# Cons-Cat/Pixel-Art-Raytracer

Measured on AMD Instinct MI355X. Metric: Mrays/sec at 4096x4096, 1024 prims, higher is better.
Workload: dtype int32+f32; 1 GPU; 4096x4096x4096 view, bin 40, 1024 primitives (splitmix64 seed 12345), light (2560,2048,1024); RGBA8 frame + palette-index plane; frames_in_flight=4, streams_overlap_pairwise=True

## Files before the change

pixel-art-raytracer_amd/csrc/par_book.cpp:

```cpp
#include "par_book.h"
#include "par_internal.h"

using S = par_book_state;

static par_footprint footprint_of(const par_book& b, const par_aabb& a) {
    const int W = b.W, H = b.H, L = b.L, B = b.B;
    par_footprint f;
    const int minx = a.px, miny = a.py, minz = a.pz;
    const int maxx = minx + a.ex, maxy = miny + a.ey, maxz = minz + a.ez;
    if ((maxx < 0) || (minx >= W) || (maxy < 0 - maxz) || (miny >= H - minz + B) || (maxz < -a.ez - B) ||
        (minz > L + B)) {
        return f;
    }
    const int x0 = std::max(0, minx / B), y0 = std::max(0, (H - maxy - maxz) / B), z0 = std::max(0, minz / B);
    const int x1 = std::min(b.gx, (maxx + B - 1) / B), y1 = std::min(b.gy, (H - miny - minz + B - 1) / B);
    const int z1 = std::min(b.gz, (maxz + B - 1) / B);
    if (x1 <= x0 || y1 <= y0 || z1 <= z0) return f;
    f.x0 = (int16_t)x0; f.x1 = (int16_t)x1; f.y0 = (int16_t)y0; f.y1 = (int16_t)y1;
    f.nz = z1 - z0;
    f.items = (int32_t)((int)a.ex * ((int)a.ey + (int)a.ez) / 64 + f.cols());
    f.px = a.px; f.ex = a.ex;
    f.row0 = H - ((int)a.py + a.ey + a.pz + a.ez);
    f.rh = (int)a.ey + (int)a.ez;
    return f;
// ... 45 lines not shown
        exact += fp[i].bound();
    }
    rebuild_hist();
}

const par_book_plan& par_book::plan(par_change kind, const par_aabb* a, int first, int n) {
    refresh(kind == par_change::UPDATE ? S::CURRENT : kind == par_change::STAGE ? S::HIST_BEHIND : S::EXTENTS_ONLY);
    par_book_plan& p = plan_;
    const bool whole = kind == par_change::SET;
    p.kind = kind; p.aabbs = a; p.first = first; p.n = n;
    par_bound ex = whole ? par_bound{0, 0, 0} : exact, et = whole ? par_bound{0, 0, 0} : extent;
    const par_aabb* old = whole ? nullptr : aabbs.data() + first;
    if (kind != par_change::ASYNC) {
        p.fp.resize((size_t)n);
        par_footprint* out = p.fp.data();
        for (int i = 0; i < n; i++) {
            const par_footprint f = footprint_of(*this, a[i]);
            out[i] = f;
            ex += f.bound();
            if (old) ex -= fp[(size_t)(first + i)].bound();
        }
    }
    for (int i = 0; i < n; i++) {
        if (old && old[i].ex == a[i].ex && old[i].ey == a[i].ey && old[i].ez == a[i].ez) continue;
        et += bound_of(*this, a[i]);
        if (old) et -= bound_of(*this, old[i]);
    }
    p.exact = ex; p.extent = et;
    if (kind == par_change::ASYNC) ex = et;
    p.need = par_bound{std::max(ex.pairs, et.pairs), std::max(ex.cols, et.cols), std::max(ex.items, et.items)};
    return p;
}

void par_book::commit() {
    par_book_plan& p = plan_;
    if (p.kind != par_change::ASYNC) exact = p.exact;
    extent = p.extent;
    if (p.kind == par_change::SET) {
        aabbs.assign(p.aabbs, p.aabbs + p.n);
        fp.swap(p.fp);
        return rebuild_hist();
    }
    std::copy(p.aabbs, p.aabbs + p.n, aabbs.begin() + p.first);
    if (p.kind == par_change::UPDATE) {
        for (int i = 0; i < p.n; i++) {
            col_hist(fp[(size_t)(p.first + i)], -1);
            col_hist(p.fp[(size_t)i], +1);
        }
    }
    if (p.kind != par_change::ASYNC) std::copy(p.fp.begin(), p.fp.begin() + p.n, fp.begin() + p.first);
    state = std::max(state, p.kind == par_change::UPDATE  ? S::CURRENT
                            : p.kind == par_change::STAGE ? S::HIST_BEHIND : S::EXTENTS_ONLY);
}

const par_bound& par_book::capture() {
    refresh(S::CURRENT);
    const int64_t pairs = exact.pairs * 2 + 4096;
    const int64_t cols_max = (int64_t)((PAR_SPRITE_W + B - 1) / B + 1) * ((PAR_SPRITE_H + B - 1) / B + 1);
    const int64_t items = (int64_t)aabbs.size() * ((int64_t)PAR_SPRITE_W * PAR_SPRITE_H / 64 + cols_max);
    return graph = par_bound{pairs, pairs, std::min(items, max_items())};
}

int64_t par_book::items_per_shard(int64_t items, int64_t cols) const {
    cols = std::min<int64_t>(cols, (int64_t)gx * gy);
    return std::min(items, (cols / PAR_ITEM_SHARDS + 1) * tile_chunks());
}
```

pixel-art-raytracer_amd/csrc/par_book.h:

```cpp
#ifndef PAR_BOOK_H
#define PAR_BOOK_H

#include <stdint.h>
#include <algorithm>
#include <vector>

#include "par_raytracer.h"

struct par_bound {
    int64_t pairs, cols, items;
    par_bound& operator+=(const par_bound& b) { pairs += b.pairs; cols += b.cols; items += b.items; return *this; }
    par_bound& operator-=(const par_bound& b) { pairs -= b.pairs; cols -= b.cols; items -= b.items; return *this; }
};

struct par_footprint {
    int16_t x0 = 0, x1 = 0, y0 = 0, y1 = 0;
    int32_t nz = 0;
    int32_t items = 0;
    int16_t px = 0, ex = 0;
    int32_t row0 = 0, rh = 0;
    int32_t cols() const { return (x1 - x0) * (y1 - y0); }
    par_bound bound() const { return par_bound{(int64_t)cols() * nz, cols(), items}; }
};

enum class par_book_state : uint8_t { CURRENT, HIST_BEHIND, EXTENTS_ONLY };

enum class par_change : uint8_t { SET, UPDATE, STAGE, ASYNC };

struct par_book_plan {
    par_change kind = par_change::SET;
    const par_aabb* aabbs = nullptr; int first = 0, n = 0;
    par_bound exact{}, extent{};
    par_bound need{};
    std::vector<par_footprint> fp;
};

struct par_book {
    int W = 0, H = 0, L = 0, B = 0, gx = 0, gy = 0, gz = 0;
    par_book_state state = par_book_state::CURRENT;
    std::vector<par_aabb> aabbs;
    std::vector<par_footprint> fp;
    par_bound exact{};
    par_bound extent{};
    par_bound graph{};
    std::vector<int32_t> colpairs;
    int64_t cols_over = 0;
    std::vector<int32_t> colchunks;
    int64_t cols_tileable = 0;
    par_book_plan plan_;

    void init(const par_params& p, int x, int y, int z) {
        W = p.width; H = p.height; L = p.length; B = p.bin_size; gx = x; gy = y; gz = z;
    }
    const par_book_plan& plan(par_change kind, const par_aabb* a, int first, int n);
    void commit();
    void refresh(par_book_state lag);
    const par_bound& capture();
    void col_hist(const par_footprint& f, int sign);
    void rebuild_hist();

    par_bound frame_bounds(bool graph_mode) const {
        return graph_mode ? graph : state == par_book_state::EXTENTS_ONLY ? extent : exact;
    }
    bool may_overflow() const { return cols_over > 0 || state != par_book_state::CURRENT; }
    bool dense() const { return cols_tileable >= std::max<int64_t>(16, (int64_t)gx * gy / 64); }
    int64_t chunks() const { return std::min(exact.items, max_items()); }
    int64_t tile_chunks() const { return ((int64_t)B * B + 63) / 64; }
    int64_t max_items() const { return (int64_t)gx * gy * tile_chunks(); }
    int64_t items_per_shard(int64_t items, int64_t cols) const;
};

#endif
```

pixel-art-raytracer_amd/csrc/par_context.hip:

```cpp
#include <algorithm>
#include <array>
#include <cmath>
#include <new>
#include <cstdio>
#include <cstdlib>
#include <cstring>
#include <string>
#include <unordered_map>
#include <vector>

#include "par_book.h"
#include "par_hostcall.h"
#include "par_internal.h"

struct par_context {
    par_params params{};
    int device = 0;
    int gx = 0, gy = 0, gz = 0, volume = 0;
    hipStream_t stream = nullptr;

    par_book book;
    int n_entities = 0, n_sprites = 0, max_sprite_id = 0;
    bool have_entities = false;
    par_light lights[PAR_MAX_LIGHTS]{};
    int n_lights = 0;
    int depth_min = 0, depth_max = 0;
    int light_model = PAR_LIGHTS_UNBOUNDED;
    bool tinted = false;
    par_light_tints tints{};
    int set = 0;
    struct {
        bool valid = false;
        int r0 = 0, r1 = 0, set = 0;
        bool host_gbuf = false;
    } kept;
    struct {
        bool valid = false;
        const void* fb = nullptr;
        const void* palidx = nullptr;
        int r0 = 0, r1 = 0, set = 0;
    } drawn;
    hipStream_t last_stream = nullptr;
    bool has_last_stream = false;

    par_aabb* d_aabbs = nullptr;
    int32_t* d_sprite_ids = nullptr;
    par_sprite* d_sprites = nullptr;
    par_color* d_palette = nullptr;
    par_texel* d_texinfo = nullptr;
    unsigned long long* d_ray_counter = nullptr;
    uint8_t* d_scratch_lit = nullptr;
    size_t scratch_lit_bytes = 0;
    par_grid_dev grid{};
    int aabb_capacity = 0;

    uint8_t* d_out[5] = {nullptr, nullptr, nullptr, nullptr, nullptr};
    size_t d_out_bytes[5] = {0, 0, 0, 0, 0};

    hipGraphExec_t graph_exec[2] = {nullptr, nullptr};
    hipGraph_t graph[2] = {nullptr, nullptr};
    par_aabb* pin_aabbs[2] = {nullptr, nullptr};
    int pin_aabbs_capacity[2] = {0, 0};
    par_lights_block* pin_lights[2] = {nullptr, nullptr};
    hipEvent_t ev_graph[2] = {nullptr, nullptr};
    bool ev_graph_pending[2] = {false, false};
    int stage_lo[2] = {0, 0}, stage_hi[2] = {0, 0};
    int dev_lo = 0, dev_hi = 0;
    par_aabb* pin_update = nullptr;
    int pin_update_capacity = 0;
    hipEvent_t ev_update = nullptr;
    bool ev_update_pending = false;
    hipStream_t update_stream = nullptr;
    bool graph_lights = false;
    par_lights_block* d_lights = nullptr;
// ... 44 lines not shown

void test_alloc_hook(const par_context* c) {
    if (c->hooks & PAR_HOOK_BAD_ALLOC) throw std::bad_alloc();
}

template <class F>
int guarded(par_context* ctx, F&& body) noexcept {
    try {
        return body();
    } catch (const std::bad_alloc&) {
        return fail(ctx, PAR_ERR_OOM, "host allocation failed");
    } catch (...) {
        return fail(ctx, PAR_ERR_HIP, "unexpected C++ exception");
    }
}

void retain_frame(par_context* c, int row_begin, int row_end, int set, bool host_gbuf) {
    c->kept.valid = true;
    c->kept.r0 = row_begin;
    c->kept.r1 = row_end;
    c->kept.set = set;
    c->kept.host_gbuf = host_gbuf;
}
void drop_retained(par_context* c) { c->kept.valid = false; }

void record_drawn(par_context* c, const par_outputs& out, int row_begin, int row_end, int set) {
    c->drawn.valid = true;
    c->drawn.fb = out.fb;
    c->drawn.palidx = out.palidx;
    c->drawn.r0 = row_begin;
    c->drawn.r1 = row_end;
    c->drawn.set = set;
}
void drop_drawn(par_context* c) { c->drawn.valid = false; }

int hip_fail(par_context* c, hipError_t e, const char* what) {
    return fail(c, e == hipErrorOutOfMemory ? PAR_ERR_OOM : PAR_ERR_HIP,
                std::string(what) + ": " + hipGetErrorString(e));
}

#define PAR_HIP(call)                                        \
    do {                                                     \
        hipError_t e_ = (call);                              \
        if (e_ != hipSuccess) return hip_fail(ctx, e_, #call); \
    } while (0)

bool extent_ok(const par_aabb& a) {
    return a.ex >= 0 && a.ey >= 0 && a.ez >= 0 && a.ex <= PAR_SPRITE_W && (int)a.ey + (int)a.ez <= PAR_SPRITE_H;
}

int check_update(par_context* ctx, const par_aabb* aabbs, int first, int n, bool null_ok) {
    if (first < 0 || n < 0 || !ctx->have_entities || first + n > ctx->n_entities || (!aabbs && !(null_ok && n == 0))) {
        return fail(ctx, PAR_ERR_INVALID_ARG, null_ok ? "stage range" : "update range outside the uploaded entities");
    }
    for (int i = 0; i < n; i++) {
        if (!extent_ok(aabbs[i])) return fail(ctx, PAR_ERR_EXTENT, "extent needs 0<=ex<=20, ey,ez>=0, ey+ez<=40");
    }
    return PAR_OK;
}

template <class T>
hipError_t reallocate(T** p, size_t n, bool pinned = false) {
    if (*p) {
        const hipError_t e = pinned ? hipHostFree(*p) : hipFree(*p);
        if (e != hipSuccess) return e;
    }
    *p = nullptr;
// ... 222 lines not shown
    }
    return PAR_OK;
}

int enqueue_lights_frame(par_context* ctx, hipStream_t stream, const par_bin_args& b, const par_render_args& r,
                         const par_bound& bound, bool graph_mode, bool apart, hipEvent_t* ev) {
    const par_light_state lights = make_light_state(ctx, graph_mode);
    const int rc = enqueue_build(ctx, stream, b, bound.pairs, &r, nullptr, apart);
    if (rc != PAR_OK) return rc;
    if (ev) {
        PAR_HIP(hipEventRecord(ev[EV_BUILT], stream));
        PAR_HIP(hipEventRecord(ev[EV_COLUMNS], stream));
    }
    if (r.trace_bg) PAR_HIP(par_launch_bglights(ctx->grid, r, lights, stream));
    PAR_HIP(par_launch_fill(ctx->grid, r, stream));
    if (ev) PAR_HIP(hipEventRecord(ev[EV_FILLED], stream));
    PAR_HIP(par_launch_render_lights(ctx->grid, r, lights, bound.cols, stream));
    if (ev) {
        PAR_HIP(hipEventRecord(ev[EV_ITEMS], stream));
        PAR_HIP(hipEventRecord(ev[EV_RENDERED], stream));
        PAR_HIP(hipEventRecord(ev[EV_END], stream));
        ctx->timed_tiles = false;
        ctx->timed_overflow = false;
        ctx->timed_both = false;
    }
    return PAR_OK;
}

int enqueue_frame(par_context* ctx, hipStream_t stream, int set, int row_begin, int row_end, const par_outputs& out,
                  unsigned flags, bool graph_mode, hipEvent_t* ev) {
    const bool drawn_match = ctx->drawn.valid && ctx->drawn.fb == out.fb && ctx->drawn.palidx == out.palidx &&
                             ctx->drawn.r0 == row_begin && ctx->drawn.r1 == row_end && ctx->drawn.set == (set ^ 1);
    drop_retained(ctx);
    drop_drawn(ctx);
    par_outputs outs = out;
    if ((flags & PAR_RENDER_TRACE_BACKGROUND) && !outs.lit) {
        const size_t need = (size_t)(row_end - row_begin) * ctx->params.width;
        if (ctx->scratch_lit_bytes < need) {
            if (graph_mode) return fail(ctx, PAR_ERR_NOT_READY, "render once with PAR_RENDER_TRACE_BACKGROUND before capturing it");
            PAR_HIP(grow(&ctx->d_scratch_lit, &ctx->scratch_lit_bytes, need));
        }
        outs.lit = ctx->d_scratch_lit;
    }
    if (ctx->ev_update_pending && ctx->update_stream != stream && !graph_mode) {
        PAR_HIP(hipStreamWaitEvent(stream, ctx->ev_update, 0));
    }
    if (ctx->dev_hi > ctx->dev_lo && !graph_mode) {
        PAR_HIP(hipMemcpyAsync(ctx->d_aabbs + ctx->dev_lo, ctx->book.aabbs.data() + ctx->dev_lo,
                               (size_t)(ctx->dev_hi - ctx->dev_lo) * sizeof(par_aabb), hipMemcpyHostToDevice, stream));
        ctx->dev_lo = ctx->dev_hi = 0;
    }
    par_bin_args b = make_bin_args(ctx, set, row_begin, row_end, flags);
    par_render_args r = make_render_args(ctx, set, row_begin, row_end, outs, flags, graph_mode);
    const bool apart = ev && !(flags & PAR_RENDER_TIMED_AS_LAUNCHED);
    const par_bound bound = ctx->book.frame_bounds(graph_mode);
    if ((flags & PAR_RENDER_COUNT_RAYS) && !graph_mode) {
        PAR_HIP(hipMemsetAsync(ctx->d_ray_counter, 0, 3 * sizeof(unsigned long long), stream));
    }
    if (ev) PAR_HIP(hipEventRecord(ev[EV_START], stream));
    if (graph_mode ? ctx->graph_lights : lights_path(ctx)) {
        return enqueue_lights_frame(ctx, stream, b, r, bound, graph_mode, apart, ev);
    }
    const bool may_overflow = graph_mode || ctx->book.may_overflow() || r.dense || apart;
    r.overflow_launched = may_overflow ? 1 : 0;
    par_fill_plan plan;
    const bool ride = !apart && par_plan_fill(r, &plan);
    const int64_t tiles_in_rows = (int64_t)ctx->gx * (r.by_hi - r.by_lo + 1);
    const bool kept_frame = (flags & PAR_RENDER_KEPT_OUTPUTS) && drawn_match && !graph_mode && ride && r.B % 8 == 0 &&
                            std::min(bound.cols, tiles_in_rows) * 100 <= tiles_in_rows * kKeptMaxTilesPct;
    b.kept = kept_frame ? 1 : 0;
    par_render_args rf = r;
    rf.out.lit = nullptr;
    const int rc = enqueue_build(ctx, stream, b, bound.pairs, &rf, ride && !kept_frame ? &plan : nullptr, apart);
    if (rc != PAR_OK) return rc;
    if (ev) PAR_HIP(hipEventRecord(ev[EV_BUILT], stream));
    if (ride) {
        PAR_HIP(par_launch_columns_fill(ctx->grid, rf, bound.cols, plan, kept_frame, ctx->col_roles, stream));
    } else {
        PAR_HIP(par_launch_columns(ctx->grid, r, bound.cols, ctx->col_roles, stream));
    }
    if (ev) PAR_HIP(hipEventRecord(ev[EV_COLUMNS], stream));
    if (!ride) {
        PAR_HIP(par_launch_fill(ctx->grid, r, stream));
    } else if (r.out.lit) {
        par_render_args rl = r;
        rl.out.fb = nullptr;
        rl.out.palidx = nullptr;
        PAR_HIP(par_launch_fill(ctx->grid, rl, stream));
    }
    if (ev) PAR_HIP(hipEventRecord(ev[EV_FILLED], stream));
    const int64_t item_cap_rows = ctx->book.max_items() / ctx->gy * (r.by_hi - r.by_lo + 1);
    const int64_t item_bound = std::min(bound.items, item_cap_rows);
    bool both = false;
    if (!apart) {
        const hipError_t e = par_launch_render_both(ctx->grid, r, bound.cols, item_bound, may_overflow, stream);
        if (e == hipSuccess) {
            both = true;
        } else if (e != hipErrorNotSupported) {
            return hip_fail(ctx, e, "par_launch_render_both");
        }
    }
    if (!both) {
        PAR_HIP(par_launch_render(ctx->grid, r, item_bound, stream));
        if (ev) PAR_HIP(hipEventRecord(ev[EV_ITEMS], stream));
        PAR_HIP(par_launch_render_tiles(ctx->grid, r, item_bound, stream));
    } else if (ev) {
        PAR_HIP(hipEventRecord(ev[EV_ITEMS], stream));
    }
    if (ev) PAR_HIP(hipEventRecord(ev[EV_RENDERED], stream));
// ... 10 lines not shown
int render_to_host(par_context* ctx, int row_begin, int row_end, const par_outputs* host_out, unsigned flags) {
    int rc = frame_prologue(ctx, host_out, row_begin, row_end, flags);
    if (rc != PAR_OK) return rc;
    void* host[5] = {host_out->fb, host_out->gbuf, host_out->palidx, host_out->brightness, host_out->lit};
    const size_t n = (size_t)(row_end - row_begin) * ctx->params.width;
    void* dev[5];
    for (int i = 0; i < 5; i++) {
        dev[i] = nullptr;
        if (!host[i]) continue;
        const size_t bytes = n * kPlaneElem[i];
        if (ctx->d_out_bytes[i] < bytes) PAR_HIP(grow(&ctx->d_out[i], &ctx->d_out_bytes[i], bytes));
        dev[i] = ctx->d_out[i];
    }
    par_outputs d{(par_color*)dev[0], (par_pixel*)dev[1], (uint8_t*)dev[2], (float*)dev[3], (uint8_t*)dev[4]};
    rc = enqueue_frame(ctx, ctx->stream, ctx->set, row_begin, row_end, d, flags, false, nullptr);
    if (rc != PAR_OK) return rc;
    ctx->set ^= 1;
    ctx->last_flags = flags;
    for (int i = 0; i < 5; i++) {
        if (host[i]) PAR_HIP(hipMemcpyAsync(host[i], dev[i], n * kPlaneElem[i], hipMemcpyDeviceToHost, ctx->stream));
    }
    PAR_HIP(hipStreamSynchronize(ctx->stream));
    rc = check_device_error(ctx);
    if (rc == PAR_OK) retain_frame(ctx, row_begin, row_end, ctx->set ^ 1, host_out->gbuf != nullptr);
    return rc;
}

struct par_dev_buffer {
    void** ptr;
    size_t bytes;
    int fill;
};

std::array<par_dev_buffer, 20> dev_buffers(par_context* c, bool stamps) {
    par_grid_dev& g = c->grid;
    const size_t vol = (size_t)c->volume, cols = (size_t)c->gx * c->gy, i32 = sizeof(int32_t);
    return {{
        {(void**)&g.head[0], vol * i32, -1},
        {(void**)&g.head[1], vol * i32, -1},
        {(void**)&g.count[0], vol, -1},
        {(void**)&g.count[1], vol, -1},
        {(void**)&g.colflag[0], cols * i32, -1},
        {(void**)&g.colflag[1], cols * i32, -1},
        {(void**)&g.col_list, cols * i32, -1},
        {(void**)&g.slow_list, cols * i32, -1},
        {(void**)&g.clear_list, cols * i32, -1},
        {(void**)&g.counters, PAR_CNT_TOTAL * i32, -1},
        {(void**)&g.node_counter, 2 * i32, -1},
        {(void**)&g.build_sync, 64 * i32, 0},
        {(void**)&g.item_counters, (size_t)PAR_ITEM_LISTS * PAR_ITEM_SHARDS * PAR_ITEM_COUNTER_STRIDE * i32, 0},
        {(void**)&g.stamps, stamps ? (size_t)PAR_STAMP_ROWS * PAR_STAMP_WGS * PAR_STAMP_SLOTS * sizeof(unsigned long long) : 0, 0},
        {(void**)&g.bgwalk, (size_t)c->gx * sizeof(par_bgwalk), -1},
        {(void**)&g.bglit, (size_t)c->params.width + 64, 1},
        {(void**)&g.slots, vol * PAR_SLOTS * sizeof(par_slot), 0},
        {(void**)&c->d_palette, PAR_MAX_PALETTE * sizeof(par_color), -1},
        {(void**)&c->d_ray_counter, 3 * sizeof(unsigned long long), -1},
        {(void**)&c->d_lights, sizeof(par_lights_block), -1},
    }};
}

}

int par_select_device(int* device) {
    int ndev = 0;
    if (hipGetDeviceCount(&ndev) != hipSuccess || ndev <= 0) return PAR_ERR_NO_DEVICE;
    if (*device < 0) {
        if (hipGetDevice(device) != hipSuccess) return PAR_ERR_NO_DEVICE;
    }
    if (*device >= ndev) return PAR_ERR_INVALID_ARG;
    hipDeviceProp_t prop;
    if (hipGetDeviceProperties(&prop, *device) != hipSuccess) return PAR_ERR_NO_DEVICE;
    if (std::strncmp(prop.gcnArchName, "gfx950", 6) != 0) return PAR_ERR_NO_DEVICE;
    return PAR_OK;
}

extern "C" {

const char* par_last_error(const par_context* ctx) { return ctx ? ctx->err.c_str() : ""; }

// ... 74 lines not shown
                     ctx->d_out[0], ctx->d_out[1], ctx->d_out[2], ctx->d_out[3], ctx->d_out[4]};
    for (void* p : grown) {
        if (p) (void)hipFree(p);
    }
    if (ctx->pin_update) (void)hipHostFree(ctx->pin_update);
    if (ctx->ev_update) (void)hipEventDestroy(ctx->ev_update);
    for (int s = 0; s < 2; s++) {
        if (ctx->pin_aabbs[s]) (void)hipHostFree(ctx->pin_aabbs[s]);
        if (ctx->pin_lights[s]) (void)hipHostFree(ctx->pin_lights[s]);
        if (ctx->ev_graph[s]) (void)hipEventDestroy(ctx->ev_graph[s]);
    }
    for (hipEvent_t ev : ctx->ev) {
        if (ev) (void)hipEventDestroy(ev);
    }
    if (ctx->stream) (void)hipStreamDestroy(ctx->stream);
    delete ctx;
}

static int par_set_sprites_impl(par_context* ctx, const par_sprite* sprites, int n_sprites) {
    if (!ctx || !sprites || n_sprites <= 0) return fail(ctx, PAR_ERR_INVALID_ARG, "sprites");
    test_alloc_hook(ctx);
    for (int s = 0; s < n_sprites; s++) {
        for (int t = 0; t < PAR_SPRITE_TEXELS; t++) {
            const int c = sprites[s].color[t];
            if (c < 0 || c >= ctx->params.palette_size) {
                return fail(ctx, PAR_ERR_SPRITE_ID, "sprite palette index outside the palette");
            }
        }
    }
    PAR_HIP(hipSetDevice(ctx->device));
    PAR_HIP(hipDeviceSynchronize());
    drop_graphs(ctx);
    drop_retained(ctx);
    ctx->n_sprites = 0;
    PAR_HIP(reallocate(&ctx->d_sprites, (size_t)n_sprites));
    PAR_HIP(hipMemcpy(ctx->d_sprites, sprites, (size_t)n_sprites * sizeof(par_sprite), hipMemcpyHostToDevice));
    std::vector<par_texel> tex((size_t)n_sprites * PAR_SPRITE_TEXELS);
    for (int s = 0; s < n_sprites; s++) {
        for (int t = 0; t < PAR_SPRITE_TEXELS; t++) {
            const par_color pc = ctx->params.palette[sprites[s].color[t]];
            par_texel& x = tex[(size_t)s * PAR_SPRITE_TEXELS + t];
            x.nx = sprites[s].normal[t].x; x.ny = sprites[s].normal[t].y; x.nz = sprites[s].normal[t].z;
            x.rgba = (uint32_t)pc.red | ((uint32_t)pc.green << 8) | ((uint32_t)pc.blue << 16) | ((uint32_t)pc.alpha << 24);
        }
    }
    PAR_HIP(reallocate(&ctx->d_texinfo, tex.size()));
    PAR_HIP(hipMemcpy(ctx->d_texinfo, tex.data(), tex.size() * sizeof(par_texel), hipMemcpyHostToDevice));
    int dmin = INT32_MAX, dmax = INT32_MIN;
    for (int s = 0; s < n_sprites; s++) {
        for (int t = 0; t < PAR_SPRITE_TEXELS; t++) {
            dmin = std::min(dmin, (int)sprites[s].depth[t]);
            dmax = std::max(dmax, (int)sprites[s].depth[t]);
        }
    }
    ctx->depth_min = std::max(dmin, -(1 << 24));
    ctx->depth_max = std::min(dmax, 1 << 24);
    ctx->n_sprites = n_sprites;
    return PAR_OK;
}

static int par_set_entities_impl(par_context* ctx, const par_aabb* aabbs, const int32_t* sprite_ids, int n) {
    if (!ctx || n < 0 || (n > 0 && !aabbs)) return fail(ctx, PAR_ERR_INVALID_ARG, "entities");
    test_alloc_hook(ctx);
    int max_id = 0;
    for (int i = 0; i < n; i++) {
        if (!extent_ok(aabbs[i])) {
// ... 708 lines not shown
```

pixel-art-raytracer_amd/csrc/par_internal.h:

```cpp
#ifndef PAR_INTERNAL_H
#define PAR_INTERNAL_H

#include <hip/hip_runtime.h>
#include <stdint.h>

#include "par_raytracer.h"

struct par_slot {
    int16_t px, py, pz;
    int16_t ex, ey, ez;
    int32_t entity;
};
static_assert(sizeof(par_slot) == 16, "slot record must stay 16 bytes");

constexpr int PAR_STAMP_SLOTS = 8;
constexpr int PAR_STAMP_WGS = 8192;
constexpr int PAR_STAMP_ROWS = 6;

constexpr int PAR_MAX_GRID_DIM = 1024;
constexpr int PAR_COL_NB = 32;
constexpr int PAR_COL_ENT = 64;
constexpr int PAR_BIN_WALK = 64;
constexpr int PAR_COL_WALK = 160;
constexpr int PAR_MIN_BIN = 8, PAR_MAX_BIN = 160;
// ... 98 lines not shown
constexpr int PAR_ITEM_SHARDS = 1 << PAR_ITEM_SHARD_BITS;
constexpr int PAR_ITEM_COUNTER_STRIDE = 32;
constexpr uint32_t PAR_ITEM_TILE = 0xFFFFu;
constexpr uint32_t PAR_ITEM_NONE = 0xFFFFFFFFu;
struct par_item {
    uint32_t ci;
    uint32_t visit;
    uint32_t where;
    uint32_t bins;
    par_slot entry;
};
static_assert(sizeof(par_item) == 32, "work item layout");
constexpr uint32_t PAR_ITEM_SIMPLE = 1u << 31;
constexpr uint32_t PAR_ITEM_ALONE = 1u << 30;
static_assert(PAR_MAX_GRID_DIM <= 1024 && PAR_COL_NB < 64 && PAR_MAX_BIN < 256, "the fields of an alone item");
struct par_grid_dev {
    int32_t gx, gy, gz, volume;
    int32_t* head[2];
    uint8_t* count[2];
    int32_t* colflag[2];
    par_slot* slots;
    int32_t* node_entity[2];
    int32_t* node_next[2];
    int32_t* node_bin[2];
    int32_t* node_counter;
    int32_t* col_list;
    int32_t* counters;
    par_colrec* colrec;
    par_item* items;
    int32_t* item_counters;
    int32_t* build_sync;
    int32_t* slow_list;
    int32_t* clear_list;
    par_bgwalk* bgwalk;
    uint8_t* bglit;
    unsigned long long* stamps;
    int32_t capacity;
    int32_t col_capacity;
    int32_t item_capacity;
};

struct par_bin_args {
    int32_t W, H, L, B;
    int32_t n;
    int32_t set;
    int32_t by_lo, by_hi;
    int32_t kept;
    uint32_t flags;
    int32_t test_lose_wg;
    uint32_t magic_b;
    const par_aabb* aabbs;
};

struct par_render_args {
    int32_t W, H, B;
    int32_t row_begin, row_end;
    int32_t by_lo, by_hi;
    int32_t set;
    int32_t trace_bg;
    int32_t dense;
    uint32_t magic_b;
    float ambient;
    uint32_t background;
    uint32_t flags;
    int32_t tile_k;
    uint32_t tile_k_magic;
    int32_t overflow_launched;
    par_frame_dyn dyn;
    const par_frame_dyn* dyn_ptr;
    const uint8_t* count;
    const par_slot* slots;
    const par_sprite* sprites;
    const par_texel* texinfo;
    const int32_t* sprite_ids;
    const par_color* palette;
    par_outputs out;
    unsigned long long* ray_counter;
};

enum { PAR_CNT_COLS = 0, PAR_CNT_SLOW = 1, PAR_CNT_ERROR = 2, PAR_CNT_CLEAR = 4, PAR_CNT_TOTAL = 8 };
enum { PAR_DEVERR_BARRIER = 1,
       PAR_DEVERR_OVERFLOW = 2 };

struct par_fill_plan {
    uint32_t out_rgba;
    int32_t cut[4];
};

bool par_plan_fill(const par_render_args& a, par_fill_plan* plan);
hipError_t par_launch_bin_insert(const par_grid_dev& g, const par_bin_args& a, const par_render_args* fa,
                                 const par_fill_plan* fill, hipStream_t stream);
hipError_t par_launch_build(const par_grid_dev& g, const par_bin_args& a, int64_t pair_bound, const par_render_args* fa,
                            const par_fill_plan* fill, hipStream_t stream);
hipError_t par_launch_bin_resolve(const par_grid_dev& g, const par_bin_args& a, int64_t pair_bound,
                                  const par_render_args* fa, const par_fill_plan* fill, hipStream_t stream);
hipError_t par_launch_columns(const par_grid_dev& g, const par_render_args& a, int64_t column_bound, int col_roles,
                              hipStream_t stream);
hipError_t par_launch_columns_fill(const par_grid_dev& g, const par_render_args& a, int64_t column_bound,
                                   const par_fill_plan& fill, bool clear_tiles, int col_roles, hipStream_t stream);
hipError_t par_launch_fill(const par_grid_dev& g, const par_render_args& a, hipStream_t stream);
hipError_t par_launch_render(const par_grid_dev& g, const par_render_args& a, int64_t item_bound,
                             hipStream_t stream);
hipError_t par_launch_render_tiles(const par_grid_dev& g, const par_render_args& a, int64_t item_bound,
                                   hipStream_t stream);
hipError_t par_launch_render_both(const par_grid_dev& g, const par_render_args& a, int64_t column_bound,
                                  int64_t item_bound, bool may_overflow, hipStream_t stream);
hipError_t par_launch_render_overflow(const par_grid_dev& g, const par_render_args& a, int64_t column_bound,
                                      hipStream_t stream);

hipError_t par_launch_render_lights(const par_grid_dev& g, const par_render_args& a, const par_light_state& s,
// ... 12 lines not shown
```

pixel-art-raytracer_amd/csrc/par_kernels.hip:

```cpp
#include "par_internal.h"
#include "par_fastdiv.h"
#include "par_strips.h"
#include "par_lightbox.h"

#include <limits.h>

#include <algorithm>
#include <tuple>
#include <type_traits>

namespace {

__device__ __forceinline__ void stamp(const par_grid_dev& g, uint32_t flags, int k, int i) {
    if (g.stamps && (flags & (1u << 29)) && threadIdx.x == 0 && blockIdx.x < PAR_STAMP_WGS) {
        g.stamps[((size_t)k * PAR_STAMP_WGS + blockIdx.x) * PAR_STAMP_SLOTS + i] = __builtin_amdgcn_s_memrealtime();
    }
}

__device__ __forceinline__ int flat_index(int gy, int gz, int x, int y, int z) {
    return x * gy * gz + y * gz + z;
}

template <bool COH, typename T>
__device__ __forceinline__ void st_shared(T* p, T v) {
// ... 29 lines not shown
__device__ __forceinline__ void item_arrived(u32x8& v) {
#if defined(__HIP_DEVICE_COMPILE__)
    asm volatile("s_waitcnt lgkmcnt(0)" : "+s"(v) : : "memory");
#endif
}

__device__ __forceinline__ int wave_incl_scan_i(int v, int lane) {
#if defined(__HIP_DEVICE_COMPILE__)
    (void)lane;
    v += __builtin_amdgcn_update_dpp(0, v, 0x111, 0xF, 0xF, false);
    v += __builtin_amdgcn_update_dpp(0, v, 0x112, 0xF, 0xF, false);
    v += __builtin_amdgcn_update_dpp(0, v, 0x114, 0xF, 0xF, false);
    v += __builtin_amdgcn_update_dpp(0, v, 0x118, 0xF, 0xF, false);
    v += __builtin_amdgcn_update_dpp(0, v, 0x142, 0xA, 0xF, false);
    v += __builtin_amdgcn_update_dpp(0, v, 0x143, 0xC, 0xF, false);
    return v;
#else
    for (int d = 1; d < 64; d <<= 1) {
        const int y = __shfl_up(v, d);
        if (lane >= d) v += y;
    }
    return v;
#endif
}

__device__ __forceinline__ int wave_bcast(int v, int src) { return __builtin_amdgcn_readlane(v, src); }

__device__ __forceinline__ int div_bin(int n, uint32_t magic) {
    const int q = (int)__umulhi((uint32_t)(n < 0 ? -n : n), magic);
    return n < 0 ? -q : q;
}


template <int ENT, bool COH = false>
__device__ __forceinline__ void bin_insert_body(const par_grid_dev& g, const par_bin_args& a, int block, int n_blocks) {
    const int tid = block * blockDim.x + threadIdx.x;
    const int stride = n_blocks * blockDim.x;
    const int s = a.set, o = a.set ^ 1;

    const int prev = min(g.node_counter[o], g.capacity);
    for (int i = tid; i < prev; i += stride) {
        const int b = g.node_bin[o][i];
        g.head[o][b] = 0;
        g.count[o][b] = 0;
        const int col = b / g.gz;
        if (!a.kept) {
            g.colflag[o][col] = 0;
            continue;
        }
        const int by = col % g.gy;
        if (atomicExch(&g.colflag[o][col], 0) != 0 && by >= a.by_lo && by <= a.by_hi) {
            const unsigned long long m = __ballot(1);
            const int leader = __ffsll((long long)m) - 1;
            const int wl = threadIdx.x & 63;
            int base = 0;
            if (wl == leader) base = atomicAdd(&g.counters[PAR_CNT_CLEAR + s], __popcll(m));
            base = __shfl(base, leader);
            const int at = base + __popcll(m & ((1ull << wl) - 1ull));
            if (at >= 0 && at < g.gx * g.gy) g.clear_list[at] = col;
        }
    }
    if (tid < PAR_CNT_ERROR) st_shared<COH>(&g.counters[tid], 0);
    if (tid == PAR_CNT_ERROR) st_shared<COH>(&g.counters[PAR_CNT_CLEAR + o], 0);
    if (tid < PAR_ITEM_LISTS * PAR_ITEM_SHARDS) g.item_counters[tid * PAR_ITEM_COUNTER_STRIDE] = 0;

    const int W = a.W, H = a.H, L = a.L, B = a.B;
    const int lane = threadIdx.x & 63;
    const int n_waves = stride >> 6;
    for (int e0 = (tid >> 6) * ENT; e0 < a.n; e0 += n_waves * ENT) {
        const int e = e0 + lane;
        int k = 0, org = 0, dim = 0;
        if (lane < ENT && e < a.n) {
            const par_aabb box = a.aabbs[e];
            const int minx = box.px, miny = box.py, minz = box.pz;
            const int maxx = minx + box.ex, maxy = miny + box.ey, maxz = minz + box.ez;
            const bool culled = (maxx < 0) || (minx >= W) || (maxy < 0 - maxz) || (miny >= H - minz + B) ||
                                (maxz < -box.ez - B) || (minz > L + B);
            if (!culled) {
                const uint32_t mb = a.magic_b;
                const int x0 = max(0, div_bin(minx, mb));
                const int y0 = max(0, div_bin(H - maxy - maxz, mb));
// ... 28 lines not shown
                const int ny = d3 & 0x7FF, nz = d3 >> 11;
                const int t = (int)(((float)j + 0.5f) * __builtin_amdgcn_rcpf((float)nz));
                const int jz = j - t * nz;
                const int jx = (int)(((float)t + 0.5f) * __builtin_amdgcn_rcpf((float)ny));
                const int jy = t - jx * ny;
                const int b = flat_index(g.gy, g.gz, (o3 & 0x3FF) + jx, ((o3 >> 10) & 0x3FF) + jy, (o3 >> 20) + jz);
                const int node = base + p;
                if (node < g.capacity && b >= 0 && b < g.volume) {
                    st_shared<COH>(&g.node_entity[s][node], e0 + lo);
                    st_shared<COH>(&g.node_bin[s][node], b);
                    st_shared<COH>(&g.node_next[s][node], atomicExch(&g.head[s][b], node + 1));
                }
            }
        }
    }
}

template <int ENT>
__global__ __launch_bounds__(256) void bin_insert_kernel(par_grid_dev g, par_bin_args a) {
    stamp(g, a.flags, 0, 0);
    bin_insert_body<ENT>(g, a, (int)blockIdx.x, (int)gridDim.x);
    stamp(g, a.flags, 0, 7);
}

__device__ __forceinline__ par_slot slot_of(const par_aabb& box, int entity) {
    par_slot rec;
    rec.px = box.px; rec.py = box.py; rec.pz = box.pz;
    rec.ex = box.ex; rec.ey = box.ey; rec.ez = box.ez;
    rec.entity = entity;
    return rec;
}

template <bool COH>
__device__ __forceinline__ void bin_resolve_node(const par_grid_dev& g, const par_bin_args& a, int tid) {
    const int s = a.set;
    const int b = ld_shared<COH>(&g.node_bin[s][tid]);
    if (ld_shared<COH>(&g.head[s][b]) != tid + 1) return;

    int top0 = -1, top1 = -1, top2 = -1, top3 = -1, top4 = -1, top5 = -1, top6 = -1;
    int k = 0;
    for (int cur = tid + 1; cur != 0; cur = ld_shared<COH>(&g.node_next[s][cur - 1])) {
        int e = ld_shared<COH>(&g.node_entity[s][cur - 1]);
        int t;
        if (e > top0) { t = top0; top0 = e; e = t; }
        if (e > top1) { t = top1; top1 = e; e = t; }
        if (e > top2) { t = top2; top2 = e; e = t; }
        if (e > top3) { t = top3; top3 = e; e = t; }
        if (e > top4) { t = top4; top4 = e; e = t; }
        if (e > top5) { t = top5; top5 = e; e = t; }
        if (e > top6) { t = top6; top6 = e; e = t; }
        k++;
    }
    const int c = k & (PAR_SLOTS - 1);
    const int top[7] = {top0, top1, top2, top3, top4, top5, top6};
#pragma unroll
    for (int i = 0; i < 7; i++) {
        if (i < c) {
            const int e = top[i];
            g.slots[(size_t)b * PAR_SLOTS + (c - 1 - i)] = slot_of(a.aabbs[e], e);
        }
    }
    g.count[s][b] = (uint8_t)c;
    if (c > 0) {
        const int col = b / g.gz;
        const int by = col % g.gy;
        if (atomicExch(&g.colflag[s][col], 1) == 0 && by >= a.by_lo && by <= a.by_hi) {
            const unsigned long long m = __ballot(1);
            const int leader = __ffsll((long long)m) - 1;
            const int lane = threadIdx.x & 63;
            int base = 0;
            if (lane == leader) base = atomicAdd(&g.counters[PAR_CNT_COLS], __popcll(m));
            base = __shfl(base, leader);
            g.col_list[base + __popcll(m & ((1ull << lane) - 1ull))] = col;
        }
    }
}

template <bool COH = false>
__device__ __forceinline__ void bin_resolve_body(const par_grid_dev& g, const par_bin_args& a, int block, int n_blocks) {
    const int tid0 = block * blockDim.x + threadIdx.x;
    const int s = a.set;
    if (tid0 == 0) g.node_counter[s ^ 1] = 0;
    const int n_nodes = min(ld_shared<COH>(&g.node_counter[s]), g.capacity);
    for (int tid = tid0; tid < n_nodes; tid += n_blocks * blockDim.x) bin_resolve_node<COH>(g, a, tid);
}

__global__ __launch_bounds__(256) void bin_resolve_kernel(par_grid_dev g, par_bin_args a) {
    stamp(g, a.flags, 1, 0);
    bin_resolve_body(g, a, (int)blockIdx.x, (int)gridDim.x);
    stamp(g, a.flags, 1, 7);
}


__device__ __forceinline__ float std_min(float a, float b) { return (b < a) ? b : a; }
__device__ __forceinline__ float std_max(float a, float b) { return (a < b) ? b : a; }

template <bool FINITE = false>
__device__ __forceinline__ bool slab_hit(const par_slot& r, int ox, int oy, int oz, float ix, float iy, float iz) {
    const float x1 = (float)(r.px - ox) * ix;
    const float x2 = (float)(r.px + r.ex - ox) * ix;
    const float y1 = (float)(r.py - oy) * iy;
    const float y2 = (float)(r.py + r.ey - oy) * iy;
    const float z1 = (float)(r.pz - oz) * iz;
    const float z2 = (float)(r.pz + r.ez - oz) * iz;
    if (FINITE) {
        const float tmin = __builtin_fmaxf(__builtin_fmaxf(__builtin_fminf(x1, x2), __builtin_fminf(y1, y2)), __builtin_fminf(z1, z2));
        const float tmax = __builtin_fminf(__builtin_fminf(__builtin_fmaxf(x1, x2), __builtin_fmaxf(y1, y2)), __builtin_fmaxf(z1, z2));
        return tmax >= tmin;
    }
    float tmin = std_min(x1, x2);
    float tmax = std_max(x1, x2);
    tmin = std_max(tmin, std_min(y1, y2));
    tmax = std_min(tmax, std_max(y1, y2));
    tmin = std_max(tmin, std_min(z1, z2));
    tmax = std_min(tmax, std_max(z1, z2));
    return tmax >= tmin;
}
// ... 622 lines not shown
                }
            }
        }
        if (a.out.palidx) {
            const int x = x0 + lane * 8;
            if (x < W) {
                typedef uint32_t u32x2 __attribute__((ext_vector_type(2)));
                const u32x2 v = {0xFFFFFFFFu, 0xFFFFFFFFu};
                __builtin_nontemporal_store(v, reinterpret_cast<u32x2*>(a.out.palidx + rowbase + x));
            }
        }
        if (a.out.lit) {
            const int x = x0 + lane * 8;
            if (x < W) {
                typedef uint32_t u32x2 __attribute__((ext_vector_type(2)));
                __builtin_nontemporal_store(*reinterpret_cast<const u32x2*>(bglit + x),
                                            reinterpret_cast<u32x2*>(a.out.lit + rowbase + x));
            }
        }
    }
}

__device__ __forceinline__ void clear_tiles_body(const par_grid_dev& g, const par_render_args& a, uint32_t out_rgba,
                                                 int block, int n_blocks) {
    const int W = a.W, B = a.B;
    const int lane = threadIdx.x & 63;
    const int wpb = blockDim.x >> 6;
    const int n_all = g.gx * g.gy;
    const int n = min(ld_uniform(&g.counters[PAR_CNT_CLEAR + a.set]), n_all);
    uint32_t* fb = reinterpret_cast<uint32_t*>(a.out.fb);
    for (int t = __builtin_amdgcn_readfirstlane(block * wpb + ((int)threadIdx.x >> 6)); t < n; t += n_blocks * wpb) {
        const int col = ld_uniform(&g.clear_list[t]);
        if (col < 0 || col >= n_all) continue;
        const int bx = col / g.gy, by = col - bx * g.gy;
        const int x0 = bx * B, x1 = min(x0 + B, W);
        const int y0 = max(by * B, a.row_begin), y1 = min(by * B + B, a.row_end);
        const int w = x1 - x0;
        if (w <= 0 || y0 >= y1) continue;
        if (fb) {
            const int lpr = w >> 2, rpi = 64 / lpr;
            const int r = lane / lpr, xi = lane - r * lpr;
            if (r < rpi) {
                typedef uint32_t u32x4 __attribute__((ext_vector_type(4)));
                const u32x4 v = {out_rgba, out_rgba, out_rgba, out_rgba};
                for (int y = y0 + r; y < y1; y += rpi) {
                    *reinterpret_cast<u32x4*>(fb + (size_t)(y - a.row_begin) * W + x0 + xi * 4) = v;
                }
            }
        }
        if (a.out.palidx) {
            const int lpr = w >> 3, rpi = 64 / lpr;
            const int r = lane / lpr, xi = lane - r * lpr;
            if (r < rpi) {
                typedef uint32_t u32x2 __attribute__((ext_vector_type(2)));
                const u32x2 v = {0xFFFFFFFFu, 0xFFFFFFFFu};
                for (int y = y0 + r; y < y1; y += rpi) {
                    *reinterpret_cast<u32x2*>(a.out.palidx + (size_t)(y - a.row_begin) * W + x0 + xi * 8) = v;
                }
            }
        }
    }
}

__global__ __launch_bounds__(256) void fill_kernel(par_render_args a, uint32_t out_rgba, const uint8_t* bglit) {
    fill_body(a, out_rgba, bglit, (int)blockIdx.x, (int)gridDim.x, make_int2(0, -1));
}
// ... 1845 lines not shown
```

Measured before the change: 1.737 million Mrays/s.

## Track dirty primitive ranges to skip redraw of unchanged frames and clean tiles

```diff
diff --git a/pixel-art-raytracer_amd/csrc/par_book.cpp b/pixel-art-raytracer_amd/csrc/par_book.cpp
--- a/pixel-art-raytracer_amd/csrc/par_book.cpp
+++ b/pixel-art-raytracer_amd/csrc/par_book.cpp
@@ -101,8 +101,44 @@
     return p;
 }
 
+void par_dirty_set::add(int first, int count) {
+    if (count <= 0) return;
+    int32_t a = first, b = first + count;
+    int m = 0;
+    for (int i = 0; i < n; i++) {
+        if (hi[i] < a || lo[i] > b) {
+            lo[m] = lo[i];
+            hi[m++] = hi[i];
+        } else {
+            a = std::min(a, lo[i]);
+            b = std::max(b, hi[i]);
+        }
+    }
+    int at = m;
+    for (; at > 0 && lo[at - 1] > a; at--) {
+        lo[at] = lo[at - 1];
+        hi[at] = hi[at - 1];
+    }
+    lo[at] = a;
+    hi[at] = b;
+    n = m + 1;
+    if (n <= MAX) return;
+    int best = 0;
+    for (int i = 1; i + 1 < n; i++) {
+        if (lo[i + 1] - hi[i] < lo[best + 1] - hi[best]) best = i;
+    }
+    hi[best] = hi[best + 1];
+    for (int i = best + 1; i + 1 < n; i++) {
+        lo[i] = lo[i + 1];
+        hi[i] = hi[i + 1];
+    }
+    n--;
+}
+
 void par_book::commit() {
     par_book_plan& p = plan_;
+    if (p.kind == par_change::SET) dirty.mark_all();
+    else dirty.add(p.first, p.n);
     if (p.kind != par_change::ASYNC) exact = p.exact;
     extent = p.extent;
     if (p.kind == par_change::SET) {
diff --git a/pixel-art-raytracer_amd/csrc/par_book.h b/pixel-art-raytracer_amd/csrc/par_book.h
--- a/pixel-art-raytracer_amd/csrc/par_book.h
+++ b/pixel-art-raytracer_amd/csrc/par_book.h
@@ -35,6 +35,24 @@
     std::vector<par_footprint> fp;
 };
 
+struct par_dirty_set {
+    static constexpr int MAX = 4;
+    static constexpr int32_t END = INT32_MAX;
+    int n = 0;
+    int32_t lo[MAX + 1] = {}, hi[MAX + 1] = {};
+    void add(int first, int count);
+    void mark_all() { n = 1; lo[0] = 0; hi[0] = END; }
+    void clear() { n = 0; }
+    bool empty() const { return n == 0; }
+    bool all() const { return n == 1 && lo[0] == 0 && hi[0] == END; }
+    bool has(int e) const {
+        for (int i = 0; i < n; i++) {
+            if (e >= lo[i] && e < hi[i]) return true;
+        }
+        return false;
+    }
+};
+
 struct par_book {
     int W = 0, H = 0, L = 0, B = 0, gx = 0, gy = 0, gz = 0;
     par_book_state state = par_book_state::CURRENT;
@@ -47,6 +65,7 @@
     int64_t cols_over = 0;
     std::vector<int32_t> colchunks;
     int64_t cols_tileable = 0;
+    par_dirty_set dirty;
     par_book_plan plan_;
 
     void init(const par_params& p, int x, int y, int z) {
diff --git a/pixel-art-raytracer_amd/csrc/par_context.hip b/pixel-art-raytracer_amd/csrc/par_context.hip
--- a/pixel-art-raytracer_amd/csrc/par_context.hip
+++ b/pixel-art-raytracer_amd/csrc/par_context.hip
@@ -40,6 +40,7 @@
         const void* palidx = nullptr;
         int r0 = 0, r1 = 0, set = 0;
     } drawn;
+    uint32_t frame_seq = 0;
     hipStream_t last_stream = nullptr;
     bool has_last_stream = false;
 
@@ -150,7 +151,10 @@
     c->drawn.r1 = row_end;
     c->drawn.set = set;
 }
-void drop_drawn(par_context* c) { c->drawn.valid = false; }
+void drop_drawn(par_context* c) {
+    c->drawn.valid = false;
+    c->book.dirty.mark_all();
+}
 
 int hip_fail(par_context* c, hipError_t e, const char* what) {
     return fail(c, e == hipErrorOutOfMemory ? PAR_ERR_OOM : PAR_ERR_HIP,
@@ -439,7 +443,11 @@
     const bool drawn_match = ctx->drawn.valid && ctx->drawn.fb == out.fb && ctx->drawn.palidx == out.palidx &&
                              ctx->drawn.r0 == row_begin && ctx->drawn.r1 == row_end && ctx->drawn.set == (set ^ 1);
     drop_retained(ctx);
+    if (ctx->dev_hi > ctx->dev_lo && !graph_mode) ctx->book.dirty.add(ctx->dev_lo, ctx->dev_hi - ctx->dev_lo);
+    const par_dirty_set dirty = ctx->book.dirty;
     drop_drawn(ctx);
+    ctx->book.dirty.clear();
+    if (++ctx->frame_seq == 0) ctx->frame_seq = 1;
     par_outputs outs = out;
     if ((flags & PAR_RENDER_TRACE_BACKGROUND) && !outs.lit) {
         const size_t need = (size_t)(row_end - row_begin) * ctx->params.width;
@@ -459,6 +467,7 @@
     }
     par_bin_args b = make_bin_args(ctx, set, row_begin, row_end, flags);
     par_render_args r = make_render_args(ctx, set, row_begin, row_end, outs, flags, graph_mode);
+    r.seq = ctx->frame_seq;
     const bool apart = ev && !(flags & PAR_RENDER_TIMED_AS_LAUNCHED);
     const par_bound bound = ctx->book.frame_bounds(graph_mode);
     if ((flags & PAR_RENDER_COUNT_RAYS) && !graph_mode) {
@@ -473,15 +482,29 @@
     par_fill_plan plan;
     const bool ride = !apart && par_plan_fill(r, &plan);
     const int64_t tiles_in_rows = (int64_t)ctx->gx * (r.by_hi - r.by_lo + 1);
-    const bool kept_frame = (flags & PAR_RENDER_KEPT_OUTPUTS) && drawn_match && !graph_mode && ride && r.B % 8 == 0 &&
+    const bool keepable = (flags & PAR_RENDER_KEPT_OUTPUTS) && drawn_match && !graph_mode && ride && r.B % 8 == 0;
+    const bool unchanged_frame = keepable && dirty.empty();
+    const bool kept_frame = keepable && !unchanged_frame &&
                             std::min(bound.cols, tiles_in_rows) * 100 <= tiles_in_rows * kKeptMaxTilesPct;
     b.kept = kept_frame ? 1 : 0;
+    static_assert(par_dirty_set::MAX == 4, "par_dirty_dev holds four ranges");
+    if (kept_frame) {
+        b.dirty.seq = r.seq;
+        b.dirty.n = dirty.n;
+        for (int i = 0; i < dirty.n && i < 4; i++) {
+            b.dirty.lo[i] = dirty.lo[i];
+            b.dirty.len[i] = (uint32_t)(dirty.hi[i] - dirty.lo[i]);
+        }
+    }
     par_render_args rf = r;
     rf.out.lit = nullptr;
-    const int rc = enqueue_build(ctx, stream, b, bound.pairs, &rf, ride && !kept_frame ? &plan : nullptr, apart);
+    const bool fills = ride && !kept_frame && !unchanged_frame;
+    const int rc = enqueue_build(ctx, stream, b, bound.pairs, &rf, fills ? &plan : nullptr, apart);
     if (rc != PAR_OK) return rc;
     if (ev) PAR_HIP(hipEventRecord(ev[EV_BUILT], stream));
-    if (ride) {
+    if (unchanged_frame) {
+        PAR_HIP(par_launch_columns(ctx->grid, rf, bound.cols, ctx->col_roles, stream));
+    } else if (ride) {
         PAR_HIP(par_launch_columns_fill(ctx->grid, rf, bound.cols, plan, kept_frame, ctx->col_roles, stream));
     } else {
         PAR_HIP(par_launch_columns(ctx->grid, r, bound.cols, ctx->col_roles, stream));
@@ -558,7 +581,7 @@
     int fill;
 };
 
-std::array<par_dev_buffer, 20> dev_buffers(par_context* c, bool stamps) {
+std::array<par_dev_buffer, 21> dev_buffers(par_context* c, bool stamps) {
     par_grid_dev& g = c->grid;
     const size_t vol = (size_t)c->volume, cols = (size_t)c->gx * c->gy, i32 = sizeof(int32_t);
     return {{
@@ -571,6 +594,7 @@
         {(void**)&g.col_list, cols * i32, -1},
         {(void**)&g.slow_list, cols * i32, -1},
         {(void**)&g.clear_list, cols * i32, -1},
+        {(void**)&g.coldirty, cols * i32, 0},
         {(void**)&g.counters, PAR_CNT_TOTAL * i32, -1},
         {(void**)&g.node_counter, 2 * i32, -1},
         {(void**)&g.build_sync, 64 * i32, 0},
@@ -711,6 +735,7 @@
     PAR_HIP(hipDeviceSynchronize());
     drop_graphs(ctx);
     drop_retained(ctx);
+    ctx->book.dirty.mark_all();
     ctx->n_sprites = 0;
     PAR_HIP(reallocate(&ctx->d_sprites, (size_t)n_sprites));
     PAR_HIP(hipMemcpy(ctx->d_sprites, sprites, (size_t)n_sprites * sizeof(par_sprite), hipMemcpyHostToDevice));
diff --git a/pixel-art-raytracer_amd/csrc/par_internal.h b/pixel-art-raytracer_amd/csrc/par_internal.h
--- a/pixel-art-raytracer_amd/csrc/par_internal.h
+++ b/pixel-art-raytracer_amd/csrc/par_internal.h
@@ -154,12 +154,20 @@
     int32_t* build_sync;
     int32_t* slow_list;
     int32_t* clear_list;
+    int32_t* coldirty;
     par_bgwalk* bgwalk;
     uint8_t* bglit;
     unsigned long long* stamps;
     int32_t capacity;
     int32_t col_capacity;
     int32_t item_capacity;
+};
+
+struct par_dirty_dev {
+    uint32_t seq;
+    int32_t n;
+    int32_t lo[4];
+    uint32_t len[4];
 };
 
 struct par_bin_args {
@@ -172,6 +180,7 @@
     int32_t test_lose_wg;
     uint32_t magic_b;
     const par_aabb* aabbs;
+    par_dirty_dev dirty;
 };
 
 struct par_render_args {
@@ -198,6 +207,7 @@
     const par_color* palette;
     par_outputs out;
     unsigned long long* ray_counter;
+    uint32_t seq;
 };
 
 enum { PAR_CNT_COLS = 0, PAR_CNT_SLOW = 1, PAR_CNT_ERROR = 2, PAR_CNT_CLEAR = 4, PAR_CNT_TOTAL = 8 };
diff --git a/pixel-art-raytracer_amd/csrc/par_kernels.hip b/pixel-art-raytracer_amd/csrc/par_kernels.hip
--- a/pixel-art-raytracer_amd/csrc/par_kernels.hip
+++ b/pixel-art-raytracer_amd/csrc/par_kernels.hip
@@ -85,13 +85,19 @@
 }
 
 
+__device__ __forceinline__ bool dirty_entity(const par_dirty_dev& d, int e) {
+    return ((uint32_t)(e - d.lo[0]) < d.len[0]) | ((uint32_t)(e - d.lo[1]) < d.len[1]) |
+           ((uint32_t)(e - d.lo[2]) < d.len[2]) | ((uint32_t)(e - d.lo[3]) < d.len[3]);
+}
+
 template <int ENT, bool COH = false>
 __device__ __forceinline__ void bin_insert_body(const par_grid_dev& g, const par_bin_args& a, int block, int n_blocks) {
     const int tid = block * blockDim.x + threadIdx.x;
     const int stride = n_blocks * blockDim.x;
     const int s = a.set, o = a.set ^ 1;
 
-    const int prev = min(g.node_counter[o], g.capacity);
+    const int prev_all = g.node_counter[o];
+    const int prev = min(prev_all, g.capacity);
     for (int i = tid; i < prev; i += stride) {
         const int b = g.node_bin[o][i];
         g.head[o][b] = 0;
@@ -100,6 +106,9 @@
         if (!a.kept) {
             g.colflag[o][col] = 0;
             continue;
+        }
+        if (a.dirty.n > 0 && (prev_all > g.capacity || dirty_entity(a.dirty, g.node_entity[o][i]))) {
+            g.coldirty[col] = (int32_t)a.dirty.seq;
         }
         const int by = col % g.gy;
         if (atomicExch(&g.colflag[o][col], 0) != 0 && by >= a.by_lo && by <= a.by_hi) {
@@ -194,15 +203,18 @@
 }
 
 template <bool COH>
-__device__ __forceinline__ void bin_resolve_node(const par_grid_dev& g, const par_bin_args& a, int tid) {
+__device__ __forceinline__ void bin_resolve_node(const par_grid_dev& g, const par_bin_args& a, int tid, bool lost) {
     const int s = a.set;
     const int b = ld_shared<COH>(&g.node_bin[s][tid]);
     if (ld_shared<COH>(&g.head[s][b]) != tid + 1) return;
 
     int top0 = -1, top1 = -1, top2 = -1, top3 = -1, top4 = -1, top5 = -1, top6 = -1;
     int k = 0;
+    const bool marks = a.dirty.n > 0;
+    bool rewritten = lost;
     for (int cur = tid + 1; cur != 0; cur = ld_shared<COH>(&g.node_next[s][cur - 1])) {
         int e = ld_shared<COH>(&g.node_entity[s][cur - 1]);
+        if (marks) rewritten |= dirty_entity(a.dirty, e);
         int t;
         if (e > top0) { t = top0; top0 = e; e = t; }
         if (e > top1) { t = top1; top1 = e; e = t; }
@@ -223,6 +235,7 @@
         }
     }
     g.count[s][b] = (uint8_t)c;
+    if (marks && rewritten) g.coldirty[b / g.gz] = (int32_t)a.dirty.seq;
     if (c > 0) {
         const int col = b / g.gz;
         const int by = col % g.gy;
@@ -243,8 +256,9 @@
     const int tid0 = block * blockDim.x + threadIdx.x;
     const int s = a.set;
     if (tid0 == 0) g.node_counter[s ^ 1] = 0;
-    const int n_nodes = min(ld_shared<COH>(&g.node_counter[s]), g.capacity);
-    for (int tid = tid0; tid < n_nodes; tid += n_blocks * blockDim.x) bin_resolve_node<COH>(g, a, tid);
+    const int n_all = ld_shared<COH>(&g.node_counter[s]);
+    const int n_nodes = min(n_all, g.capacity);
+    for (int tid = tid0; tid < n_nodes; tid += n_blocks * blockDim.x) bin_resolve_node<COH>(g, a, tid, n_all > g.capacity);
 }
 
 __global__ __launch_bounds__(256) void bin_resolve_kernel(par_grid_dev g, par_bin_args a) {
@@ -933,6 +947,7 @@
     for (int t = __builtin_amdgcn_readfirstlane(block * wpb + ((int)threadIdx.x >> 6)); t < n; t += n_blocks * wpb) {
         const int col = ld_uniform(&g.clear_list[t]);
         if (col < 0 || col >= n_all) continue;
+        if (ld_uniform(&g.coldirty[col]) != (int32_t)a.seq) continue;
         const int bx = col / g.gy, by = col - bx * g.gy;
         const int x0 = bx * B, x1 = min(x0 + B, W);
         const int y0 = max(by * B, a.row_begin), y1 = min(by * B + B, a.row_end);
```

New measurement: 2.107 million Mrays/s (median of 6 runs). 1.21x the previous value.
